# gopi-erabati/SRFDet3D

Measured on AMD Instinct MI355X. Metric: frames/sec, srfdet_voxel_nusc_LC synthetic 30k-pt sweeps, higher is better.
Workload: dtype f32

## Files before the change

include/srfdet3d.h:

```cpp
#ifndef SRFDET3D_H
#define SRFDET3D_H

#include <stddef.h>
#include <stdint.h>

#ifdef __cplusplus
extern "C" {
#endif

typedef void *srf_stream_t;

#define SRF_OK 0
#define SRF_EINVAL (-1)
#define SRF_EWORKSPACE (-2)
#define SRF_EUNSUPPORTED (-3)
#define SRF_EHIP_BASE (-1000)

int srf_abi_version(void);
const char *srf_error_string(int code);
int srf_device_count(void);

size_t srf_bitmap_words(const int *shape, int batch);
size_t srf_bitmap_pair_count_ints(void);
size_t srf_bitmap_workspace_bytes(size_t words);
int srf_bitmap_build(const int *indices, int A, const int *shape, int batch, void *bitmap, int *prefix, int *order,
                     int *sorted_indices, void *workspace, size_t workspace_bytes, srf_stream_t stream);
int srf_bitmap_build_padded(const int *indices, int A, const int *shape, int batch, void *bitmap, int *prefix, int *order,
                            int *sorted_indices, void *workspace, size_t workspace_bytes, srf_stream_t stream);
int srf_bitmap_rulebook_subm(const int *sorted_indices, int A, const int *shape, int batch, const int *ksize,
                             const void *bitmap, const int *prefix, int *nbr , int *pair_counts ,
                             srf_stream_t stream);
int srf_bitmap_strided_outputs(const int *indices, int A, const int *shape, int batch, const int *ksize, const int *stride,
                               const int *pad, void *out_bitmap, int *out_prefix, int *out_indices, int out_capacity,
                               int *num_out, void *workspace, size_t workspace_bytes, srf_stream_t stream);
int srf_bitmap_strided_outputs_static(const int *indices, int A, const int *shape, int batch, const int *ksize, const int *stride,
                                      const int *pad, void *out_bitmap, int *out_prefix, int *out_indices, int out_capacity,
                                      int *num_out, void *workspace, size_t workspace_bytes, srf_stream_t stream);
int srf_bitmap_strided_pairs(const int *out_indices, const int *num_out, int max_out, const int *shape, int batch,
                             const int *ksize, const int *stride, const int *pad, const void *in_bitmap, const int *in_prefix,
                             int in_rows, int *nbr, int nbr_stride, int fill_tail, int *pair_counts, srf_stream_t stream);

int srf_densify_bev(const float *feats, int A, int C, const void *bitmap, const int *prefix, int B, int D, int H, int W, float *out,
                    srf_stream_t stream);

int srf_pillar_vfe(const float *voxels, const int *num, const int *coors4, const int *rows_dev, int rows, int P, int nf,
                   const float *voxel_size , const float *offset , int cluster_center, int voxel_center, int legacy,
                   const float *W, const float *scale, const float *shift, int Cout, float *out, srf_stream_t stream);
// ... 342 lines not shown
```

srfdet3d_amd/_lib.py:

```python
import ctypes
import os
from ctypes import POINTER, c_char_p, c_float, c_int, c_int64, c_longlong, c_size_t, c_void_p

_HERE = os.path.dirname(os.path.abspath(__file__))
LIB_PATH = os.path.join(_HERE, "libsrfdet3d_hip.so")

_lib = None


class FeatMap(ctypes.Structure):
    _fields_ = [("data", c_void_p), ("N", c_int), ("H", c_int), ("W", c_int),
                ("stride_n", c_int64), ("stride_c", c_int64), ("stride_h", c_int64), ("stride_w", c_int64),
                ("spatial_scale", c_float)]


_P = c_void_p
_HF = POINTER(c_float)
_HI = POINTER(c_int)

SIGNATURES = {
    "srf_abi_version": (c_int, []),
    "srf_error_string": (c_char_p, [c_int]),
    "srf_device_count": (c_int, []),
    "srf_points_filter_workspace_bytes": (c_size_t, [c_int]),
# ... 39 lines not shown
    "srf_conv_wgrad_nhwc": (c_int, [_P, c_int64, _P, c_int64, c_int, c_int, c_int, c_int, c_int, c_int, _P, c_size_t, _P, _P]),
    "srf_spconv_tiles_count": (c_int, [c_int]),
    "srf_spconv_tiles_row_cost": (c_int, []),
    "srf_spconv_tiles_workspace_bytes": (c_size_t, [c_int]),
    "srf_spconv_tiles_build": (c_int, [_P, c_int, c_int, c_int, _P, _P, _P, _P]),
    "srf_spconv_order_ints": (c_size_t, [c_int, c_int]),
    "srf_spconv_order_build": (c_int, [_P, c_int, c_int, c_int, _P, _P, _P]),
    "srf_spconv_bf16_packed_weight_bytes": (c_size_t, [c_int, c_int, c_int]),
    "srf_spconv_bf16_pack_weights": (c_int, [_P, c_int, c_int, c_int, _P, _P]),
    "srf_spconv_fwd_bf16": (c_int, [_P, c_int, c_int, _P, c_int, _P, c_int, c_int, c_int, _P, _P, _P, c_int, _P, _P, _P, _P]),
    "srf_densify": (c_int, [_P, _P, c_int, c_int, c_int, c_int, c_int, c_int, _P, c_int, _P]),
    "srf_roi_extract": (c_int, [POINTER(FeatMap), c_int, c_int, _P, c_int, c_int, c_int, c_float, _P, c_int64,
                                c_int64, c_int64, c_int, _P, _P]),
    "srf_roi_extract_sum": (c_int, [POINTER(FeatMap), c_int, c_int, _P, c_int, c_int, c_int, c_int, c_float, _P, c_int64, c_int64, c_int64, _P]),
    "srf_linear_workspace_bytes": (c_size_t, [c_int, c_int, c_int]),
    "srf_linear": (c_int, [_P, c_int, c_int, c_int, _P, c_int, c_int, _P, _P, _P, c_float, c_int, _P, c_int, _P, _P, c_float,
                           c_int, _P, c_int, _P, c_size_t, _P]),
    "srf_self_attention": (c_int, [_P, c_int, c_int, c_int, _P, _P]),
    "srf_self_attention_batched": (c_int, [_P, c_int, c_int, c_int, c_int, _P, _P]),
    "srf_dynconv_mid": (c_int, [_P, _P, c_int, c_int, c_int, c_int, _P, _P, c_float, _P, _P, c_float, _P, _P]),
    "srf_bitmap_words": (c_size_t, [_HI, c_int]),
    "srf_bitmap_pair_count_ints": (c_size_t, []),
    "srf_bitmap_workspace_bytes": (c_size_t, [c_size_t]),
    "srf_bitmap_build": (c_int, [_P, c_int, _HI, c_int, _P, _P, _P, _P, _P, c_size_t, _P]),
    "srf_densify_bev": (c_int, [_P, c_int, c_int, _P, _P, c_int, c_int, c_int, c_int, _P, _P]),
    "srf_pillar_vfe": (c_int, [_P, _P, _P, _P, c_int, c_int, c_int, _HF, _HF, c_int, c_int, c_int, _P, _P, _P, c_int, _P, _P]),
    "srf_pillar_scatter_nhwc": (c_int, [_P, _P, _P, c_int, c_int, c_int, c_int, c_int, _P, _P]),
    "srf_dvfe_workspace_bytes": (c_size_t, [c_int, c_int]),
    "srf_dvfe_fwd": (c_int, [_P, c_int, c_int, _P, _P, _P, _P, _P, _P, c_int, _HF, _HF, c_int, _P, _P, _P, _P, _P, _P, c_int, _P, _P, _P,
                             c_int, _P, _P, _P, c_int, _P, _P, c_size_t, _P]),
    "srf_bitmap_build_padded": (c_int, [_P, c_int, _HI, c_int, _P, _P, _P, _P, _P, c_size_t, _P]),
    "srf_bitmap_rulebook_subm": (c_int, [_P, c_int, _HI, c_int, _HI, _P, _P, _P, _P, _P]),
    "srf_bitmap_strided_outputs": (c_int, [_P, c_int, _HI, c_int, _HI, _HI, _HI, _P, _P, _P, c_int, _P, _P, c_size_t, _P]),
    "srf_bitmap_strided_outputs_static": (c_int, [_P, c_int, _HI, c_int, _HI, _HI, _HI, _P, _P, _P, c_int, _P, _P, c_size_t, _P]),
    "srf_bitmap_strided_pairs": (c_int, [_P, _P, c_int, _HI, c_int, _HI, _HI, _HI, _P, _P, c_int, _P, c_int, c_int, _P, _P]),
    "srf_upsample_add": (c_int, [_P, _P, c_int, c_int, c_int, c_int, c_int, _P, _P]),
    "srf_maxpool3s2_ceil": (c_int, [_P, c_int, c_int, c_int, _P, _P]),
    "srf_ese_gate": (c_int, [_P, c_int, c_int, _P, _P, _P, _P]),
    "srf_nchw_to_nhwc": (c_int, [_P, c_int, c_int, c_int, _P, _P]),
    "srf_dwconv3x3s2": (c_int, [_P, c_int, c_int, c_int, c_int, _P, _P, _P, c_int, _P, _P]),
    "srf_channel_affine": (c_int, [_P, c_int, c_int, c_int, c_longlong, _P, _P, c_int, _P, c_int, _P, c_longlong, _P]),
    "srf_conv1x1_packed_weight_bytes": (c_size_t, [c_int, c_int]),
    "srf_conv1x1_pack_weights": (c_int, [_P, c_int, c_int, _P, _P]),
    "srf_conv1x1": (c_int, [POINTER(c_void_p), _HI, c_int, c_int, c_int, _P, c_int, _P, _P, c_int, _P, _P]),
    "srf_wino43_packed_weight_bytes": (c_size_t, [c_int, c_int]),
    "srf_wino43_pack_weights": (c_int, [_P, c_int, c_int, _P, _P]),
# ... 124 lines not shown
```

srfdet3d_amd/csrc/common.hpp:

```cpp
#pragma once
#include <hip/hip_runtime.h>
#include <stdint.h>
#include <stdlib.h>

#include "../../include/srfdet3d.h"

#define SRF_WAVE 64

#define SRF_HIP_TRY(expr)                                    \
    do {                                                     \
        hipError_t _e = (expr);                              \
        if (_e != hipSuccess) return SRF_EHIP_BASE - (int)_e; \
    } while (0)

#define SRF_LAUNCH_CHECK()                                   \
    do {                                                     \
        hipError_t _e = hipGetLastError();                   \
        if (_e != hipSuccess) return SRF_EHIP_BASE - (int)_e; \
    } while (0)

static inline int srf_ceil_div(long long a, long long b) { return (int)((a + b - 1) / b); }
static inline size_t srf_align256(size_t x) { return (x + 255) & ~(size_t)255; }

static inline long long srf_knob(const char *name, long long dflt)
// ... 107 lines not shown
    return v;
}

__device__ __forceinline__ int srf_block_exclusive_scan_256(int v, int *total, int *lds4 )
{
    const int lane = threadIdx.x & 63, wave = threadIdx.x >> 6;
    int inc = srf_wave_inclusive_scan(v);
    if (lane == 63) lds4[wave] = inc;
    __syncthreads();
    int w0 = lds4[0], w1 = lds4[1], w2 = lds4[2], w3 = lds4[3];
    int base = (wave > 0 ? w0 : 0) + (wave > 1 ? w1 : 0) + (wave > 2 ? w2 : 0);
    *total = w0 + w1 + w2 + w3;
    __syncthreads();
    return base + inc - v;
}

#define SRF_SCAN_THREADS 256
#define SRF_SCAN_ITEMS 8
#define SRF_SCAN_TILE (SRF_SCAN_THREADS * SRF_SCAN_ITEMS)

static inline int srf_scan_blocks(long long n) { return n > 0 ? srf_ceil_div(n, SRF_SCAN_TILE) : 1; }

template <class ValF>
__global__ __launch_bounds__(SRF_SCAN_THREADS) void srf_scan_reduce_k(int n, ValF val, int *__restrict__ partial)
{
    __shared__ int lds[4];
    const int base = blockIdx.x * SRF_SCAN_TILE;
    int s = 0;
#pragma unroll
    for (int j = 0; j < SRF_SCAN_ITEMS; ++j) {
        int i = base + j * SRF_SCAN_THREADS + threadIdx.x;
        if (i < n) s += val(i);
    }
    s = srf_wave_sum(s);
    if ((threadIdx.x & 63) == 0) lds[threadIdx.x >> 6] = s;
    __syncthreads();
    if (threadIdx.x == 0) partial[blockIdx.x] = lds[0] + lds[1] + lds[2] + lds[3];
}

static __global__ __launch_bounds__(256) void srf_scan_partials_k(int nb, int *__restrict__ partial, int *__restrict__ total_out,
                                                         int clamp_max)
{
    __shared__ int lds[4];
    int carry = 0;
    for (int base = 0; base < nb; base += 256) {
        int i = base + threadIdx.x;
        int v = i < nb ? partial[i] : 0;
        int tot;
        int ex = srf_block_exclusive_scan_256(v, &tot, lds);
        if (i < nb) partial[i] = carry + ex;
        carry += tot;
    }
    if (threadIdx.x == 0) {
        partial[nb] = carry;
        if (total_out) *total_out = (clamp_max >= 0 && carry > clamp_max) ? clamp_max : carry;
    }
}

template <class ValF, class OutF>
__global__ __launch_bounds__(SRF_SCAN_THREADS) void srf_scan_apply_k(int n, ValF val, const int *__restrict__ partial,
                                                                   OutF out)
{
    __shared__ int lds[4];
    const int base = blockIdx.x * SRF_SCAN_TILE + threadIdx.x * SRF_SCAN_ITEMS;
    int v[SRF_SCAN_ITEMS];
    int s = 0;
#pragma unroll
    for (int j = 0; j < SRF_SCAN_ITEMS; ++j) {
        int i = base + j;
        v[j] = i < n ? val(i) : 0;
        s += v[j];
    }
    int tot;
    int ex = srf_block_exclusive_scan_256(s, &tot, lds) + partial[blockIdx.x];
#pragma unroll
    for (int j = 0; j < SRF_SCAN_ITEMS; ++j) {
        int i = base + j;
        if (i < n) out(i, v[j], ex);
        ex += v[j];
    }
}

#define SRF_SCAN_SINGLE_THREADS 1024
#define SRF_SCAN_SINGLE_MAX (SRF_SCAN_SINGLE_THREADS * SRF_SCAN_ITEMS)

template <class ValF, class OutF>
__global__ __launch_bounds__(SRF_SCAN_SINGLE_THREADS) void srf_scan_single_k(int n, ValF val, OutF out, int *__restrict__ partial_total,
                                                                           int *__restrict__ total_out, int clamp_max)
{
    __shared__ int s_w[SRF_SCAN_SINGLE_THREADS / 64];
    const int lane = threadIdx.x & 63, wave = threadIdx.x >> 6;
    int carry = 0;
    for (int base0 = 0; base0 < n; base0 += SRF_SCAN_SINGLE_THREADS * SRF_SCAN_ITEMS) {
        const int base = base0 + threadIdx.x * SRF_SCAN_ITEMS;
        int v[SRF_SCAN_ITEMS];
        int s = 0;
#pragma unroll
        for (int j = 0; j < SRF_SCAN_ITEMS; ++j) {
            const int i = base + j;
            v[j] = i < n ? val(i) : 0;
            s += v[j];
        }
        const int inc = srf_wave_inclusive_scan(s);
        if (lane == 63) s_w[wave] = inc;
        __syncthreads();
        int before = 0, tot = 0;
#pragma unroll
        for (int w = 0; w < SRF_SCAN_SINGLE_THREADS / 64; ++w) {
            const int c = s_w[w];
            before += w < wave ? c : 0;
            tot += c;
        }
        __syncthreads();
        int ex = carry + before + inc - s;
#pragma unroll
        for (int j = 0; j < SRF_SCAN_ITEMS; ++j) {
            const int i = base + j;
            if (i < n) out(i, v[j], ex);
            ex += v[j];
        }
        carry += tot;
    }
    if (threadIdx.x == 0) {
        *partial_total = carry;
        if (total_out) *total_out = (clamp_max >= 0 && carry > clamp_max) ? clamp_max : carry;
    }
}

template <class ValF, class OutF>
static inline int srf_device_scan(int n, ValF val, OutF out, int *partial, int *total_out, int clamp_max,
                                  hipStream_t st)
{
    const int nb = srf_scan_blocks(n);
    if (n <= SRF_SCAN_SINGLE_MAX) {
        hipLaunchKernelGGL(HIP_KERNEL_NAME(srf_scan_single_k<ValF, OutF>), dim3(1), dim3(SRF_SCAN_SINGLE_THREADS), 0, st, n, val, out,
                           partial + nb, total_out, clamp_max);
        SRF_LAUNCH_CHECK();
        return SRF_OK;
    }
    hipLaunchKernelGGL(HIP_KERNEL_NAME(srf_scan_reduce_k<ValF>), dim3(nb), dim3(SRF_SCAN_THREADS), 0, st, n, val, partial);
    hipLaunchKernelGGL(srf_scan_partials_k, dim3(1), dim3(256), 0, st, nb, partial, total_out, clamp_max);
    hipLaunchKernelGGL(HIP_KERNEL_NAME(srf_scan_apply_k<ValF, OutF>), dim3(nb), dim3(SRF_SCAN_THREADS), 0, st, n, val,
                       partial, out);
    SRF_LAUNCH_CHECK();
    return SRF_OK;
}
```

srfdet3d_amd/csrc/rulebook.hip:

```cpp
#include "common.hpp"

#define SRF_MAX_K 27

struct ConvGeom {
    int shape[3];
    int oshape[3];
    int ks[3], st[3], pd[3];
    int K;
};

__device__ __forceinline__ uint32_t srf_coord_key(int b, int z, int y, int x, const int *shape)
{
    return (((uint32_t)b * (uint32_t)shape[0] + (uint32_t)z) * (uint32_t)shape[1] + (uint32_t)y) * (uint32_t)shape[2] +
           (uint32_t)x;
}

__global__ __launch_bounds__(256) void srf_table_build_k(const int4 *__restrict__ indices, int A, ConvGeom g,
                                                       uint32_t *keys, int *rows, uint32_t mask)
{
    const int i = blockIdx.x * 256 + threadIdx.x;
    if (i >= A) return;
    int4 c = indices[i];
    int s = srf_table_insert(keys, mask, srf_coord_key(c.x, c.y, c.z, c.w, g.shape));
    if (s >= 0) rows[s] = i;
// ... 46 lines not shown

__global__ __launch_bounds__(256) void srf_strided_insert_k(const int4 *__restrict__ indices, int A, ConvGeom g,
                                                          uint32_t *okeys, uint32_t omask, int *mincand,
                                                          int *__restrict__ cand_slot)
{
    const long long c = (long long)blockIdx.x * 256 + threadIdx.x;
    if (c >= (long long)A * g.K) return;
    const int i = (int)(c / g.K), k = (int)(c % g.K);
    int4 ci = indices[i];
    int q[3];
    int slot = -1;
    if (srf_candidate(ci, k, g, q)) {
        slot = srf_table_insert(okeys, omask, srf_coord_key(ci.x, q[0], q[1], q[2], g.oshape));
        if (slot >= 0) atomicMin(&mincand[slot], (int)c);
    }
    cand_slot[c] = slot;
}

struct StridedFlag {
    const int *cand_slot;
    const int *mincand;
    __device__ int operator()(int c) const
    {
        int s = cand_slot[c];
        return (s >= 0 && mincand[s] == c) ? 1 : 0;
    }
};

struct StridedAssign {
    const int4 *indices;
    const int *cand_slot;
    int *orows;
    int4 *out_indices;
    ConvGeom g;
    __device__ void operator()(int c, int v, int prefix) const
    {
        if (!v) return;
        const int i = c / g.K, k = c % g.K;
        int4 ci = indices[i];
        int q[3];
        srf_candidate(ci, k, g, q);
        orows[cand_slot[c]] = prefix;
        out_indices[prefix] = make_int4(ci.x, q[0], q[1], q[2]);
    }
};

__global__ __launch_bounds__(256) void srf_strided_fill_k(int A, int K, const int *__restrict__ cand_slot,
                                                        const int *__restrict__ orows, int num_out,
// ... 358 lines not shown
        if (v >= in_rows) v = -1;
        nbr[(size_t)k * nbr_stride + o] = v;
    } else if (fill_tail && o < nbr_stride) {
        nbr[(size_t)k * nbr_stride + o] = -1;
    }
    if (pair_counts) srf_bm_count(v >= 0, k, pair_counts);
}

static long long srf_bm_cells(const int *shape, int batch)
{
    if (!shape || batch <= 0 || shape[0] <= 0 || shape[1] <= 0 || shape[2] <= 0) return -1;
    const unsigned long long c = (unsigned long long)batch * shape[0] * shape[1] * shape[2];
    return c < 0xFFFFFFFFull ? (long long)c : -1;
}

extern "C" size_t srf_bitmap_pair_count_ints(void) { return (size_t)SRF_MAX_K * (SRF_BM_REPLICAS + 1); }

extern "C" size_t srf_bitmap_words(const int *shape, int batch)
{
    const long long c = srf_bm_cells(shape, batch);
    return c < 0 ? 0 : (size_t)((c + 31) / 32);
}

extern "C" size_t srf_bitmap_workspace_bytes(size_t words) { return (size_t)(srf_scan_blocks((long long)words) + 1) * sizeof(int); }

static int srf_bitmap_build_impl(const int *indices, int A, const int *shape, int batch, void *bitmap, int *prefix, int *order,
                                 int *sorted_indices, void *workspace, size_t workspace_bytes, srf_stream_t stream, int padded)
{
    const size_t words = srf_bitmap_words(shape, batch);
    if (A < 0 || words == 0 || !bitmap || !prefix || !workspace) return SRF_EINVAL;
    if (workspace_bytes < srf_bitmap_workspace_bytes(words)) return SRF_EWORKSPACE;
    ConvGeom g;
    const int one[3] = {1, 1, 1};
    if (!srf_fill_conv_geom(g, shape, one, one, nullptr, batch)) return SRF_EINVAL;
    hipStream_t st = (hipStream_t)stream;
    SrfFillRegions fill = {};
    fill.ptr[0] = (uint32_t *)bitmap, fill.value[0] = 0u, fill.nwords[0] = words;
    if (padded && A > 0 && order && sorted_indices) {
        fill.ptr[1] = (uint32_t *)order, fill.value[1] = 0u, fill.nwords[1] = (size_t)A;
        fill.ptr[2] = (uint32_t *)sorted_indices, fill.value[2] = 0xFFFFFFFFu, fill.nwords[2] = (size_t)A * 4;
    }
    SRF_HIP_TRY(srf_fill_regions(fill, st));
    if (A > 0) {
        if (!indices) return SRF_EINVAL;
        hipLaunchKernelGGL(srf_bm_mark_k, dim3(srf_ceil_div(A, 256)), dim3(256), 0, st, (const int4 *)indices, A, g,
                           (uint32_t *)bitmap);
    }
    int rc = srf_device_scan((int)words, BmPop{(const uint32_t *)bitmap}, BmPrefix{prefix}, (int *)workspace, nullptr, -1, st);
    if (rc) return rc;
    if (A > 0 && order && sorted_indices)
        hipLaunchKernelGGL(srf_bm_place_k, dim3(srf_ceil_div(A, 256)), dim3(256), 0, st, (const int4 *)indices, A, g,
                           (const uint32_t *)bitmap, prefix, order, (int4 *)sorted_indices);
    SRF_LAUNCH_CHECK();
    return SRF_OK;
}

extern "C" int srf_bitmap_build(const int *indices, int A, const int *shape, int batch, void *bitmap, int *prefix, int *order,
                                int *sorted_indices, void *workspace, size_t workspace_bytes, srf_stream_t stream)
{
    return srf_bitmap_build_impl(indices, A, shape, batch, bitmap, prefix, order, sorted_indices, workspace, workspace_bytes, stream, 0);
}

extern "C" int srf_bitmap_build_padded(const int *indices, int A, const int *shape, int batch, void *bitmap, int *prefix, int *order,
                                       int *sorted_indices, void *workspace, size_t workspace_bytes, srf_stream_t stream)
{
    return srf_bitmap_build_impl(indices, A, shape, batch, bitmap, prefix, order, sorted_indices, workspace, workspace_bytes, stream, 1);
}

extern "C" int srf_bitmap_rulebook_subm(const int *sorted_indices, int A, const int *shape, int batch, const int *ksize,
                                        const void *bitmap, const int *prefix, int *nbr, int *pair_counts, srf_stream_t stream)
{
// ... 10 lines not shown
    if (pair_counts)
        hipLaunchKernelGGL(srf_bm_fold_counts_k, dim3(1), dim3(64), 0, st, pair_counts + SRF_MAX_K, g.K, pair_counts);
    SRF_LAUNCH_CHECK();
    return SRF_OK;
}

static int srf_bitmap_strided_outputs_impl(const int *indices, int A, const int *shape, int batch, const int *ksize,
                                           const int *stride, const int *pad, void *out_bitmap, int *out_prefix, int *out_indices,
                                           int out_capacity, int *num_out, void *workspace, size_t workspace_bytes,
                                           srf_stream_t stream, int fill_tail)
{
    ConvGeom g;
    if (A < 0 || !shape || !ksize || !stride || !pad || !num_out || !out_bitmap || !out_prefix || !workspace || out_capacity < 0)
        return SRF_EINVAL;
    if (!srf_fill_conv_geom(g, shape, ksize, stride, pad, batch)) return SRF_EINVAL;
    const size_t words = srf_bitmap_words(g.oshape, batch);
    if (words == 0) return SRF_EINVAL;
    if (workspace_bytes < srf_bitmap_workspace_bytes(words)) return SRF_EWORKSPACE;
    hipStream_t st = (hipStream_t)stream;
    SrfFillRegions fill = {};
    fill.ptr[0] = (uint32_t *)out_bitmap, fill.value[0] = 0u, fill.nwords[0] = words;
    if (fill_tail && out_indices && out_capacity > 0)
        fill.ptr[1] = (uint32_t *)out_indices, fill.value[1] = 0xFFFFFFFFu, fill.nwords[1] = (size_t)out_capacity * 4;
    SRF_HIP_TRY(srf_fill_regions(fill, st));
    if (A > 0) {
        if (!indices || !out_indices) return SRF_EINVAL;
        hipLaunchKernelGGL(srf_bm_strided_mark_k, dim3(srf_ceil_div(A, 256), g.K), dim3(256), 0, st, (const int4 *)indices, A, g,
                           (uint32_t *)out_bitmap);
    }
    int rc = srf_device_scan((int)words, BmPop{(const uint32_t *)out_bitmap}, BmPrefix{out_prefix}, (int *)workspace, num_out, -1, st);
    if (rc) return rc;
    if (A > 0)
        hipLaunchKernelGGL(srf_bm_emit_k, dim3(srf_ceil_div((long long)words, 256)), dim3(256), 0, st, (const uint32_t *)out_bitmap,
                           out_prefix, (int)words, g.oshape[0], g.oshape[1], g.oshape[2], out_capacity, (int4 *)out_indices);
    SRF_LAUNCH_CHECK();
    return SRF_OK;
}

extern "C" int srf_bitmap_strided_outputs(const int *indices, int A, const int *shape, int batch, const int *ksize,
                                          const int *stride, const int *pad, void *out_bitmap, int *out_prefix, int *out_indices,
                                          int out_capacity, int *num_out, void *workspace, size_t workspace_bytes,
                                          srf_stream_t stream)
{
    return srf_bitmap_strided_outputs_impl(indices, A, shape, batch, ksize, stride, pad, out_bitmap, out_prefix, out_indices,
                                           out_capacity, num_out, workspace, workspace_bytes, stream, 0);
}

extern "C" int srf_bitmap_strided_outputs_static(const int *indices, int A, const int *shape, int batch, const int *ksize,
                                                 const int *stride, const int *pad, void *out_bitmap, int *out_prefix,
                                                 int *out_indices, int out_capacity, int *num_out, void *workspace,
                                                 size_t workspace_bytes, srf_stream_t stream)
{
    return srf_bitmap_strided_outputs_impl(indices, A, shape, batch, ksize, stride, pad, out_bitmap, out_prefix, out_indices,
// ... 59 lines not shown
```

srfdet3d_amd/csrc/scatter.hip:

```cpp
#include "common.hpp"

struct ScatterGeom {
    int D, H, W;
    uint32_t nwords;
};

__device__ __forceinline__ bool srf_coor_key(const int4 &c, const ScatterGeom &g, uint32_t &key)
{
    if (c.x < 0 || c.y < 0 || c.z < 0 || c.w < 0) return false;
    key = (((uint32_t)c.x * (uint32_t)g.D + (uint32_t)c.y) * (uint32_t)g.H + (uint32_t)c.z) * (uint32_t)g.W + (uint32_t)c.w;
    return true;
}

__global__ __launch_bounds__(256) void srf_vu_mark_k(const int4 *__restrict__ coors, int n, ScatterGeom g,
                                                   uint32_t *bitmap)
{
    const int i = blockIdx.x * 256 + threadIdx.x;
    if (i >= n) return;
    uint32_t key;
    if (srf_coor_key(coors[i], g, key)) atomicOr(&bitmap[key >> 5], 1u << (key & 31));
}

struct VuPop {
    const uint32_t *bitmap;
// ... 103 lines not shown
    unsigned long long vol = (unsigned long long)batch;
    for (int d = 0; d < 3; ++d) {
        if (grid_zyx[d] <= 0) return false;
        vol *= (unsigned long long)grid_zyx[d];
    }
    if (vol >= 0xFFFFFFFFull) return false;
    g.D = grid_zyx[0];
    g.H = grid_zyx[1];
    g.W = grid_zyx[2];
    g.nwords = (uint32_t)((vol + 31) / 32);
    return true;
}

static size_t srf_vu_layout(int n, uint32_t nwords, size_t *o_prefix, size_t *o_cursor, size_t *o_partial)
{
    size_t b = srf_align256((size_t)nwords * 4);
    *o_prefix = b;
    b += srf_align256((size_t)nwords * 4);
    *o_cursor = b;
    b += srf_align256((size_t)(n > 0 ? n : 1) * 4);
    *o_partial = b;
    int nb = srf_scan_blocks(nwords);
    int nb2 = srf_scan_blocks(n);
    b += srf_align256((size_t)((nb > nb2 ? nb : nb2) + 1) * 4);
    return b;
}

extern "C" size_t srf_voxel_unique_workspace_bytes(int n, const int *grid_zyx, int batch)
{
    ScatterGeom g;
    if (n < 0 || !srf_scatter_geom(g, grid_zyx, batch)) return 0;
    size_t a, b, c;
    return srf_vu_layout(n, g.nwords, &a, &b, &c);
}

extern "C" int srf_voxel_unique(const int *coors, int n, const int *grid_zyx, int batch, int *out_coors,
                                int *point2voxel, int *counts, int *offsets, int *order, int *num_voxels,
                                void *workspace, size_t workspace_bytes, srf_stream_t stream)
{
    ScatterGeom g;
    if (n < 0 || !srf_scatter_geom(g, grid_zyx, batch) || !num_voxels) return SRF_EINVAL;
    hipStream_t st = (hipStream_t)stream;
    if (n == 0) {
        SRF_HIP_TRY(srf_fill_bytes(num_voxels, 0, sizeof(int), st));
        return SRF_OK;
    }
    if (!coors || !out_coors || !point2voxel || !counts || !offsets || !order || !workspace) return SRF_EINVAL;
    size_t o_prefix, o_cursor, o_partial;
    if (workspace_bytes < srf_vu_layout(n, g.nwords, &o_prefix, &o_cursor, &o_partial)) return SRF_EWORKSPACE;
    uint32_t *bitmap = (uint32_t *)workspace;
    int *prefix = (int *)((char *)workspace + o_prefix);
    int *cursor = (int *)((char *)workspace + o_cursor);
    int *partial = (int *)((char *)workspace + o_partial);

    SRF_HIP_TRY(srf_fill_bytes(bitmap, 0, (size_t)g.nwords * 4, st));
    SRF_HIP_TRY(srf_fill_bytes(cursor, 0, (size_t)n * 4, st));
    SRF_HIP_TRY(srf_fill_bytes(counts, 0, (size_t)n * 4, st));
    const int nblk = srf_ceil_div(n, 256);
    hipLaunchKernelGGL(srf_vu_mark_k, dim3(nblk), dim3(256), 0, st, (const int4 *)coors, n, g, bitmap);
    SRF_LAUNCH_CHECK();
    int rc = srf_device_scan((int)g.nwords, VuPop{bitmap}, VuEmit{bitmap, prefix, (int4 *)out_coors, g}, partial,
                             num_voxels, -1, st);
    if (rc) return rc;
    hipLaunchKernelGGL(srf_vu_map_k, dim3(nblk), dim3(256), 0, st, (const int4 *)coors, n, g, bitmap, prefix, point2voxel,
                       counts);
    SRF_LAUNCH_CHECK();
    rc = srf_device_scan(n, VuCount{counts}, VuOffset{offsets}, partial, nullptr, -1, st);
    if (rc) return rc;
    hipLaunchKernelGGL(srf_vu_place_k, dim3(nblk), dim3(256), 0, st, point2voxel, n, offsets, cursor, order);
    hipLaunchKernelGGL(srf_vu_sort_k, dim3(nblk), dim3(256), 0, st, offsets, counts, num_voxels, order);
    SRF_LAUNCH_CHECK();
    return SRF_OK;
}

extern "C" int srf_scatter_reduce(const float *feats, const int *order, const int *offsets, const int *counts,
                                  const int *num_voxels, int rows, int C, int mode, float *out, srf_stream_t stream)
{
    if (rows < 0 || C <= 0 || (mode != 0 && mode != 1) || !num_voxels) return SRF_EINVAL;
    if (rows == 0) return SRF_OK;
    if (!feats || !order || !offsets || !counts || !out) return SRF_EINVAL;
    hipLaunchKernelGGL(srf_scatter_reduce_k, dim3(srf_ceil_div((long long)rows * C, 256)), dim3(256), 0,
                       (hipStream_t)stream, feats, order, offsets, counts, num_voxels, rows, C, mode, out);
    SRF_LAUNCH_CHECK();
    return SRF_OK;
}
```

srfdet3d_amd/csrc/spconv.hip:

```cpp
#include "common.hpp"

typedef float f32x16 __attribute__((ext_vector_type(16)));
typedef float f32x4 __attribute__((ext_vector_type(4)));

#define SRF_KC 32
#define SRF_KMAX 27

template <int TM, int COUT>
__device__ __forceinline__ void srf_stage_tile(const float *__restrict__ in, int Cin, const float *__restrict__ Wk, int c0,
                                               const int *s_nbr_k, float (*s_a)[SRF_KC + 1], float (*s_w)[COUT])
{
    const int tid = threadIdx.x;
    const bool vec = (Cin & 3) == 0;
    for (int e = tid; e < TM * (SRF_KC / 4); e += 256) {
        const int r = e / (SRF_KC / 4), q = e % (SRF_KC / 4);
        const int i = s_nbr_k[r];
        const int c = c0 + q * 4;
        float4 v = make_float4(0.f, 0.f, 0.f, 0.f);
        if (i >= 0 && c < Cin) {
            const float *src = in + (size_t)i * Cin + c;
            if (vec) {
                v = *reinterpret_cast<const float4 *>(src);
            } else {
                v.x = src[0];
// ... 320 lines not shown
    }
    const int r0 = blockIdx.x * SRF_TB_ROWS;
    int carry = 0;
    for (int j = 0; j < SRF_TB_ROWS / 256; ++j) {
        const int r = r0 + j * 256 + threadIdx.x;
        int c = 0;
        {
            const int rc = r < A ? r : (A > 0 ? A - 1 : 0);
            int v[SRF_KMAX];
#pragma unroll
            for (int k = 0; k < SRF_KMAX; ++k) v[k] = nbr[(size_t)(k < K ? k : K - 1) * nbr_stride + rc];
#pragma unroll
            for (int k = 0; k < SRF_KMAX; ++k) c += (k < K && v[k] >= 0) ? 1 : 0;
            c = r < A ? c + row_cost : 0;
        }
        int total;
        const int ex = srf_block_scan_excl(c, s_scan, total);
        if (r < A) local[r] = carry + ex;
        carry += total;
    }
    if (threadIdx.x == 0) blocksum[blockIdx.x] = carry;
}

__global__ __launch_bounds__(256) void srf_gs_blockscan_k(const int *__restrict__ blocksum, int nb, int *__restrict__ blockoff)
{
    __shared__ int s_scan[4];
    int carry = 0;
    for (int b0 = 0; b0 < nb; b0 += 256) {
        const int b = b0 + threadIdx.x;
        const int v = b < nb ? blocksum[b] : 0;
        int total;
        const int ex = srf_block_scan_excl(v, s_scan, total);
        if (b < nb) blockoff[b] = carry + ex;
        carry += total;
    }
    if (threadIdx.x == 0) blockoff[nb] = carry;
}

__global__ __launch_bounds__(256) void srf_gs_cut_k(const int *__restrict__ local, const int *__restrict__ blockoff, int nb, int A,
                                                  const int *__restrict__ rows_dev, int T, int *__restrict__ tiles)
{
    if (rows_dev) {
        const int live = *rows_dev;
        A = A < live ? A : live;
    }
    const int t = blockIdx.x * 256 + threadIdx.x;
    if (t > T) return;
    const int nbl = (A + SRF_TB_ROWS - 1) / SRF_TB_ROWS;
    if (t == T || A == 0) {
        tiles[t] = A;
        return;
    }
    const long long P = blockoff[nbl];
    const long long target = (P * t + T - 1) / T;
    int lo = 0, hi = nbl - 1;
    while (lo < hi) {
        const int mid = (lo + hi + 1) >> 1;
        if (blockoff[mid] <= target) lo = mid;
        else hi = mid - 1;
    }
    const long long boff = blockoff[lo];
    const int r0 = lo * SRF_TB_ROWS;
    const int r1 = r0 + SRF_TB_ROWS < A ? r0 + SRF_TB_ROWS : A;
    int a = r0, b = r1;
    while (a < b) {
        const int mid = (a + b) >> 1;
        if (boff + local[mid] >= target) b = mid;
        else a = mid + 1;
// ... 1 lines not shown
    tiles[t] = a;
}

extern "C" int srf_spconv_tiles_count(int A_out) { return A_out <= 0 ? 1 : srf_gs_ranges(A_out); }

extern "C" int srf_spconv_tiles_row_cost(void) { return SRF_GS_ROW_BASE; }

extern "C" size_t srf_spconv_tiles_workspace_bytes(int A_out)
{
    if (A_out < 0) return 0;
    const size_t nb = (size_t)(A_out + SRF_TB_ROWS - 1) / SRF_TB_ROWS;
    return ((size_t)A_out + 2 * nb + 8) * sizeof(int);
}

extern "C" int srf_spconv_tiles_build(const int *nbr, int nbr_stride, int K, int A_out, const int *rows_dev, void *workspace,
                                      int *tiles, srf_stream_t stream)
{
    if (A_out < 0 || K <= 0 || K > SRF_KMAX || nbr_stride < A_out || !tiles) return SRF_EINVAL;
    if (A_out > 0 && (!nbr || !workspace)) return SRF_EINVAL;
    hipStream_t st = (hipStream_t)stream;
    const int T = srf_spconv_tiles_count(A_out);
    const int nb = (A_out + SRF_TB_ROWS - 1) / SRF_TB_ROWS;
    int *local = (int *)workspace, *blocksum = local + A_out, *blockoff = blocksum + nb + 1;
    if (nb > 0) {
        hipLaunchKernelGGL(srf_gs_rowpairs_k, dim3(nb), dim3(256), 0, st, nbr, nbr_stride, K, A_out, rows_dev, local, blocksum, SRF_GS_ROW_BASE);
        hipLaunchKernelGGL(srf_gs_blockscan_k, dim3(1), dim3(256), 0, st, blocksum, nb, blockoff);
    }
    hipLaunchKernelGGL(srf_gs_cut_k, dim3(srf_ceil_div(T + 1, 256)), dim3(256), 0, st, local, blockoff, nb, A_out, rows_dev, T, tiles);
    SRF_LAUNCH_CHECK();
    return SRF_OK;
}


typedef __attribute__((address_space(3))) float srf_lds_float;
typedef __attribute__((address_space(3))) f32x4 srf_lds_f32x4;
__device__ __forceinline__ unsigned srf_lds_addr(const void *p) { return (unsigned)(uintptr_t)p; }

struct SrfGspLane {
    unsigned fo0, fo1;
    unsigned sto[4];
    unsigned goff;
    unsigned colbase;
    unsigned boff;
};

struct SrfGspRegs {
    unsigned f0, f1;
    unsigned st[4];
    unsigned gaddr;
    unsigned oaddr[4];
    unsigned pin_addr;
// ... 894 lines not shown
```

srfdet3d_amd/csrc/voxelize.hip:

```cpp
#include "common.hpp"

#define SRF_SENT 0x7F7F7F7F

struct VoxelGeom {
    float vs[3];
    float lo[3];
    int grid[3];
};

__device__ __forceinline__ bool srf_point_coord(const float *p, const VoxelGeom &g, int &cx, int &cy, int &cz)
{
    int c[3];
#pragma unroll
    for (int j = 0; j < 3; ++j) {
        float d = __fsub_rn(p[j], g.lo[j]);
        float q = __fdiv_rn(d, g.vs[j]);
        float f = floorf(q);
        if (!(f >= 0.0f && f < (float)g.grid[j])) return false;
        c[j] = (int)f;
    }
    cx = c[0];
    cy = c[1];
    cz = c[2];
    return true;
// ... 43 lines not shown
    if (srf_point_coord(p, g, cx, cy, cz)) {
        uint32_t key = ((uint32_t)cz * (uint32_t)g.grid[1] + (uint32_t)cy) * (uint32_t)g.grid[0] + (uint32_t)cx;
        slot = srf_table_insert(keys, mask, key);
    }
    pslot[i] = slot;
    if (slot < 0) return;
    atomicMin(&minidx[slot], i);
    int *lst = top + (size_t)slot * max_points;
    if (i < __atomic_load_n(&lst[max_points - 1], __ATOMIC_RELAXED)) {
        int v = i;
        for (int s = 0; s < max_points; ++s) {
            int old = atomicMin(&lst[s], v);
            if (old == SRF_SENT) break;
            v = old > v ? old : v;
        }
    }
}

struct HvFlag {
    const int *pslot;
    const int *minidx;
    __device__ int operator()(int i) const
    {
        int s = pslot[i];
        return (s >= 0 && minidx[s] == i) ? 1 : 0;
    }
};

struct HvAssign {
    const int *pslot;
    const uint32_t *keys;
    int *vox_slot;
    int *coors;
    int max_voxels;
    int gx, gy;
    int cols, batch;
    __device__ void operator()(int i, int v, int prefix) const
    {
        if (!v || prefix >= max_voxels) return;
        int s = pslot[i];
        vox_slot[prefix] = s;
        uint32_t key = keys[s];
        uint32_t x = key % (uint32_t)gx;
        uint32_t t = key / (uint32_t)gx;
        int *c = coors + (size_t)cols * prefix + (cols - 3);
        if (cols == 4) c[-1] = batch;
        c[0] = (int)(t / (uint32_t)gy);
        c[1] = (int)(t % (uint32_t)gy);
// ... 60 lines not shown
                                    const int *grid, int *coors, srf_stream_t stream)
{
    if (n < 0 || nf < 3 || nf > 64 || !vs || !range || !grid) return SRF_EINVAL;
    if (n == 0) return SRF_OK;
    if (!points || !coors) return SRF_EINVAL;
    VoxelGeom g;
    if (!srf_fill_geom(g, vs, range, grid)) return SRF_EINVAL;
    hipLaunchKernelGGL(srf_dynamic_voxelize_k, dim3(srf_ceil_div(n, 256)), dim3(256), 256 * nf * sizeof(float),
                       (hipStream_t)stream, points, n, nf, g, coors);
    SRF_LAUNCH_CHECK();
    return SRF_OK;
}

extern "C" size_t srf_hard_voxelize_workspace_bytes(int n, int max_points)
{
    if (n < 0 || max_points <= 0) return 0;
    size_t cap = (size_t)srf_hv_capacity(n);
    size_t b = 0;
    b += srf_align256(cap * 4);
    b += srf_align256(cap * 4);
    b += srf_align256(cap * (size_t)max_points * 4);
    b += srf_align256((size_t)(n > 0 ? n : 1) * 4);
    b += srf_align256((size_t)(n > 0 ? n : 1) * 4);
    b += srf_align256((size_t)(srf_scan_blocks(n) + 1) * 4);
    return b;
}

static int srf_hard_voxelize_impl(const float *points, int n, int nf, const float *vs, const float *range,
                                  const int *grid, int max_points, int max_voxels, float *voxels, int *coors, int *num,
                                  int *voxel_num, float *mean, int mean_features, void *workspace,
                                  size_t workspace_bytes, srf_stream_t stream, int coor_cols, int batch_index)
{
    if (n < 0 || nf < 3 || nf > 64 || max_points <= 0 || max_points > 64 || max_voxels <= 0 || !vs || !range ||
        !grid || !voxel_num)
        return SRF_EINVAL;
    if (mean && (mean_features <= 0 || mean_features > nf)) return SRF_EINVAL;
    hipStream_t st = (hipStream_t)stream;
    if (n == 0) {
        SRF_HIP_TRY(srf_fill_bytes(voxel_num, 0, sizeof(int), st));
        return SRF_OK;
    }
    if (!points || !voxels || !coors || !num || !workspace) return SRF_EINVAL;
    if (workspace_bytes < srf_hard_voxelize_workspace_bytes(n, max_points)) return SRF_EWORKSPACE;
    VoxelGeom g;
    if (!srf_fill_geom(g, vs, range, grid)) return SRF_EINVAL;

    const size_t cap = (size_t)srf_hv_capacity(n);
    char *w = (char *)workspace;
    uint32_t *keys = (uint32_t *)w;
    w += srf_align256(cap * 4);
    int *minidx = (int *)w;
    w += srf_align256(cap * 4);
    int *top = (int *)w;
    w += srf_align256(cap * (size_t)max_points * 4);
    int *pslot = (int *)w;
    w += srf_align256((size_t)n * 4);
    int *vox_slot = (int *)w;
    w += srf_align256((size_t)n * 4);
    int *partial = (int *)w;

    SrfFillRegions fill = {};
    fill.ptr[0] = keys, fill.value[0] = 0xFFFFFFFFu, fill.nwords[0] = srf_align256(cap * 4) / 4;
    fill.ptr[1] = (uint32_t *)minidx, fill.value[1] = 0x7F7F7F7Fu;
    fill.nwords[1] = (srf_align256(cap * 4) + srf_align256(cap * (size_t)max_points * 4)) / 4;
    SRF_HIP_TRY(srf_fill_regions(fill, st));

    hipLaunchKernelGGL(srf_hv_insert_k, dim3(srf_ceil_div(n, 256)), dim3(256), 256 * nf * sizeof(float), st, points, n,
                       nf, g, max_points, keys, (uint32_t)(cap - 1), minidx, top, pslot);
    SRF_LAUNCH_CHECK();

    HvFlag flag{pslot, minidx};
    HvAssign assign{pslot, keys, vox_slot, coors, max_voxels, grid[0], grid[1], coor_cols, batch_index};
    int rc = srf_device_scan(n, flag, assign, partial, voxel_num, max_voxels, st);
    if (rc) return rc;

    const int rows = n < max_voxels ? n : max_voxels;
    const long long threads = (long long)rows * max_points * nf;
    hipLaunchKernelGGL(srf_hv_gather_k, dim3(srf_ceil_div(threads, 256)), dim3(256), 0, st, points, nf, max_points, top,
                       vox_slot, voxel_num, rows, voxels, num, mean, mean ? mean_features : 0, coor_cols == 4 ? coors : (int *)nullptr);
    SRF_LAUNCH_CHECK();
    return SRF_OK;
}

extern "C" int srf_hard_voxelize(const float *points, int n, int nf, const float *vs, const float *range,
                                 const int *grid, int max_points, int max_voxels, float *voxels, int *coors, int *num,
                                 int *voxel_num, float *mean, int mean_features, void *workspace,
                                 size_t workspace_bytes, srf_stream_t stream)
{
    return srf_hard_voxelize_impl(points, n, nf, vs, range, grid, max_points, max_voxels, voxels, coors, num, voxel_num, mean,
                                  mean_features, workspace, workspace_bytes, stream, 3, 0);
}

extern "C" int srf_hard_voxelize_static(const float *points, int n, int nf, const float *vs, const float *range,
                                        const int *grid, int max_points, int max_voxels, float *voxels, int *coors4, int *num,
                                        int *voxel_num, float *mean, int mean_features, int batch_index, void *workspace,
                                        size_t workspace_bytes, srf_stream_t stream)
// ... 6 lines not shown
```

Before: 30.35.

## Fuse scan reduce and partials via last-block ticket; merge gather-scan cut kernels

Device prefix scans now use a last-block-done atomic ticket so the reduce kernel also scans the block partials, cutting the separate partials launch. A ticket word is added to each scan workspace and cleared in the existing batched fill. The single-block path threshold drops to a tunable, lower default. Other changes: the spconv blockscan and cut kernels are merged, value loads are hoisted branch-free, the partials scan handles several items per thread, and separate memsets are batched into one fill. This trades kernel launches for atomics and redundant per-block scanning work.

```diff
diff --git a/include/srfdet3d.h b/include/srfdet3d.h
--- a/include/srfdet3d.h
+++ b/include/srfdet3d.h
@@ -23,6 +23,8 @@
 size_t srf_bitmap_words(const int *shape, int batch);
 size_t srf_bitmap_pair_count_ints(void);
 size_t srf_bitmap_workspace_bytes(size_t words);
+long long srf_scan_single_max_elements(void);
+int srf_scan_launches(long long n, long long single_max, int has_ticket);
 int srf_bitmap_build(const int *indices, int A, const int *shape, int batch, void *bitmap, int *prefix, int *order,
                      int *sorted_indices, void *workspace, size_t workspace_bytes, srf_stream_t stream);
 int srf_bitmap_build_padded(const int *indices, int A, const int *shape, int batch, void *bitmap, int *prefix, int *order,
diff --git a/srfdet3d_amd/_lib.py b/srfdet3d_amd/_lib.py
--- a/srfdet3d_amd/_lib.py
+++ b/srfdet3d_amd/_lib.py
@@ -85,6 +85,8 @@
     "srf_bitmap_words": (c_size_t, [_HI, c_int]),
     "srf_bitmap_pair_count_ints": (c_size_t, []),
     "srf_bitmap_workspace_bytes": (c_size_t, [c_size_t]),
+    "srf_scan_single_max_elements": (c_longlong, []),
+    "srf_scan_launches": (c_int, [c_longlong, c_longlong, c_int]),
     "srf_bitmap_build": (c_int, [_P, c_int, _HI, c_int, _P, _P, _P, _P, _P, c_size_t, _P]),
     "srf_densify_bev": (c_int, [_P, c_int, c_int, _P, _P, c_int, c_int, c_int, c_int, _P, _P]),
     "srf_pillar_vfe": (c_int, [_P, _P, _P, _P, c_int, c_int, c_int, _HF, _HF, c_int, c_int, c_int, _P, _P, _P, c_int, _P, _P]),
diff --git a/srfdet3d_amd/csrc/common.hpp b/srfdet3d_amd/csrc/common.hpp
--- a/srfdet3d_amd/csrc/common.hpp
+++ b/srfdet3d_amd/csrc/common.hpp
@@ -153,35 +153,89 @@
 static inline int srf_scan_blocks(long long n) { return n > 0 ? srf_ceil_div(n, SRF_SCAN_TILE) : 1; }
 
 template <class ValF>
+__device__ __forceinline__ int srf_scan_block_sum(int n, ValF &val, int *lds4)
+{
+    const int base = blockIdx.x * SRF_SCAN_TILE;
+    int v[SRF_SCAN_ITEMS];
+#pragma unroll
+    for (int j = 0; j < SRF_SCAN_ITEMS; ++j) {
+        const int i = base + j * SRF_SCAN_THREADS + threadIdx.x;
+        v[j] = val(i < n ? i : n - 1);
+    }
+    int s = 0;
+#pragma unroll
+    for (int j = 0; j < SRF_SCAN_ITEMS; ++j) s += (base + j * SRF_SCAN_THREADS + (int)threadIdx.x < n) ? v[j] : 0;
+    s = srf_wave_sum(s);
+    if ((threadIdx.x & 63) == 0) lds4[threadIdx.x >> 6] = s;
+    __syncthreads();
+    return lds4[0] + lds4[1] + lds4[2] + lds4[3];
+}
+
+template <class ValF>
 __global__ __launch_bounds__(SRF_SCAN_THREADS) void srf_scan_reduce_k(int n, ValF val, int *__restrict__ partial)
 {
     __shared__ int lds[4];
-    const int base = blockIdx.x * SRF_SCAN_TILE;
-    int s = 0;
-#pragma unroll
-    for (int j = 0; j < SRF_SCAN_ITEMS; ++j) {
-        int i = base + j * SRF_SCAN_THREADS + threadIdx.x;
-        if (i < n) s += val(i);
-    }
-    s = srf_wave_sum(s);
-    if ((threadIdx.x & 63) == 0) lds[threadIdx.x >> 6] = s;
+    const int s = srf_scan_block_sum(n, val, lds);
+    if (threadIdx.x == 0) partial[blockIdx.x] = s;
+}
+
+template <bool coherent>
+__device__ __forceinline__ int srf_scan_partials_body(int nb, int *partial, int *lds4)
+{
+    int carry = 0;
+    for (int base0 = 0; base0 < nb; base0 += SRF_SCAN_TILE) {
+        const int base = base0 + threadIdx.x * SRF_SCAN_ITEMS;
+        int v[SRF_SCAN_ITEMS];
+#pragma unroll
+        for (int j = 0; j < SRF_SCAN_ITEMS; ++j) {
+            const int *p = partial + (base + j < nb ? base + j : nb - 1);
+            v[j] = coherent ? __hip_atomic_load(p, __ATOMIC_RELAXED, __HIP_MEMORY_SCOPE_AGENT) : *p;
+        }
+        int s = 0;
+#pragma unroll
+        for (int j = 0; j < SRF_SCAN_ITEMS; ++j) {
+            v[j] = base + j < nb ? v[j] : 0;
+            s += v[j];
+        }
+        int tot;
+        int ex = carry + srf_block_exclusive_scan_256(s, &tot, lds4);
+#pragma unroll
+        for (int j = 0; j < SRF_SCAN_ITEMS; ++j) {
+            if (base + j < nb) partial[base + j] = ex;
+            ex += v[j];
+        }
+        carry += tot;
+    }
+    return carry;
+}
+
+template <class ValF>
+__global__ __launch_bounds__(SRF_SCAN_THREADS) void srf_scan_reduce_last_k(int n, ValF val, int *partial, int *ticket,
+                                                                         int *__restrict__ total_out, int clamp_max)
+{
+    __shared__ int lds[5];
+    const int s = srf_scan_block_sum(n, val, lds);
+    if (threadIdx.x == 0) {
+        __hip_atomic_store(partial + blockIdx.x, s, __ATOMIC_RELAXED, __HIP_MEMORY_SCOPE_AGENT);
+        asm volatile("s_waitcnt vmcnt(0)" ::: "memory");
+        const int t = __hip_atomic_fetch_add(ticket, 1, __ATOMIC_RELAXED, __HIP_MEMORY_SCOPE_AGENT);
+        lds[4] = t == (int)gridDim.x - 1;
+    }
     __syncthreads();
-    if (threadIdx.x == 0) partial[blockIdx.x] = lds[0] + lds[1] + lds[2] + lds[3];
-}
-
-static __global__ __launch_bounds__(256) void srf_scan_partials_k(int nb, int *__restrict__ partial, int *__restrict__ total_out,
-                                                         int clamp_max)
+    if (!lds[4]) return;
+    const int nb = (int)gridDim.x;
+    const int carry = srf_scan_partials_body<true>(nb, partial, lds);
+    if (threadIdx.x == 0) {
+        partial[nb] = carry;
+        if (total_out) *total_out = (clamp_max >= 0 && carry > clamp_max) ? clamp_max : carry;
+        __hip_atomic_store(ticket, 0, __ATOMIC_RELAXED, __HIP_MEMORY_SCOPE_AGENT);
+    }
+}
+
+static __global__ __launch_bounds__(256) void srf_scan_partials_k(int nb, int *partial, int *__restrict__ total_out, int clamp_max)
 {
     __shared__ int lds[4];
-    int carry = 0;
-    for (int base = 0; base < nb; base += 256) {
-        int i = base + threadIdx.x;
-        int v = i < nb ? partial[i] : 0;
-        int tot;
-        int ex = srf_block_exclusive_scan_256(v, &tot, lds);
-        if (i < nb) partial[i] = carry + ex;
-        carry += tot;
-    }
+    const int carry = srf_scan_partials_body<false>(nb, partial, lds);
     if (threadIdx.x == 0) {
         partial[nb] = carry;
         if (total_out) *total_out = (clamp_max >= 0 && carry > clamp_max) ? clamp_max : carry;
@@ -197,9 +251,10 @@
     int v[SRF_SCAN_ITEMS];
     int s = 0;
 #pragma unroll
+    for (int j = 0; j < SRF_SCAN_ITEMS; ++j) v[j] = val(base + j < n ? base + j : n - 1);
+#pragma unroll
     for (int j = 0; j < SRF_SCAN_ITEMS; ++j) {
-        int i = base + j;
-        v[j] = i < n ? val(i) : 0;
+        v[j] = base + j < n ? v[j] : 0;
         s += v[j];
     }
     int tot;
@@ -213,7 +268,17 @@
 }
 
 #define SRF_SCAN_SINGLE_THREADS 1024
-#define SRF_SCAN_SINGLE_MAX (SRF_SCAN_SINGLE_THREADS * SRF_SCAN_ITEMS)
+#define SRF_SCAN_SINGLE_ROUND (SRF_SCAN_SINGLE_THREADS * SRF_SCAN_ITEMS)
+#define SRF_SCAN_SINGLE_MAX_DEFAULT (5 * SRF_SCAN_SINGLE_THREADS)
+static inline long long srf_scan_single_max(void)
+{
+    static const long long v = srf_knob("SRF_SCAN_SINGLE_MAX", SRF_SCAN_SINGLE_MAX_DEFAULT);
+    return v < 0 ? 0 : v;
+}
+static inline int srf_scan_launches_for(long long n, long long single_max, int has_ticket)
+{
+    return n <= single_max ? 1 : (has_ticket ? 2 : 3);
+}
 
 template <class ValF, class OutF>
 __global__ __launch_bounds__(SRF_SCAN_SINGLE_THREADS) void srf_scan_single_k(int n, ValF val, OutF out, int *__restrict__ partial_total,
@@ -222,14 +287,15 @@
     __shared__ int s_w[SRF_SCAN_SINGLE_THREADS / 64];
     const int lane = threadIdx.x & 63, wave = threadIdx.x >> 6;
     int carry = 0;
-    for (int base0 = 0; base0 < n; base0 += SRF_SCAN_SINGLE_THREADS * SRF_SCAN_ITEMS) {
+    for (int base0 = 0; base0 < n; base0 += SRF_SCAN_SINGLE_ROUND) {
         const int base = base0 + threadIdx.x * SRF_SCAN_ITEMS;
         int v[SRF_SCAN_ITEMS];
         int s = 0;
 #pragma unroll
-        for (int j = 0; j < SRF_SCAN_ITEMS; ++j) {
-            const int i = base + j;
-            v[j] = i < n ? val(i) : 0;
+        for (int j = 0; j < SRF_SCAN_ITEMS; ++j) v[j] = val(base + j < n ? base + j : n - 1);
+#pragma unroll
+        for (int j = 0; j < SRF_SCAN_ITEMS; ++j) {
+            v[j] = base + j < n ? v[j] : 0;
             s += v[j];
         }
         const int inc = srf_wave_inclusive_scan(s);
@@ -260,17 +326,23 @@
 
 template <class ValF, class OutF>
 static inline int srf_device_scan(int n, ValF val, OutF out, int *partial, int *total_out, int clamp_max,
-                                  hipStream_t st)
+                                  hipStream_t st, int *ticket = nullptr)
 {
     const int nb = srf_scan_blocks(n);
-    if (n <= SRF_SCAN_SINGLE_MAX) {
+    const int launches = srf_scan_launches_for(n, srf_scan_single_max(), ticket != nullptr);
+    if (launches == 1) {
         hipLaunchKernelGGL(HIP_KERNEL_NAME(srf_scan_single_k<ValF, OutF>), dim3(1), dim3(SRF_SCAN_SINGLE_THREADS), 0, st, n, val, out,
                            partial + nb, total_out, clamp_max);
         SRF_LAUNCH_CHECK();
         return SRF_OK;
     }
-    hipLaunchKernelGGL(HIP_KERNEL_NAME(srf_scan_reduce_k<ValF>), dim3(nb), dim3(SRF_SCAN_THREADS), 0, st, n, val, partial);
-    hipLaunchKernelGGL(srf_scan_partials_k, dim3(1), dim3(256), 0, st, nb, partial, total_out, clamp_max);
+    if (launches == 2) {
+        hipLaunchKernelGGL(HIP_KERNEL_NAME(srf_scan_reduce_last_k<ValF>), dim3(nb), dim3(SRF_SCAN_THREADS), 0, st, n, val, partial,
+                           ticket, total_out, clamp_max);
+    } else {
+        hipLaunchKernelGGL(HIP_KERNEL_NAME(srf_scan_reduce_k<ValF>), dim3(nb), dim3(SRF_SCAN_THREADS), 0, st, n, val, partial);
+        hipLaunchKernelGGL(srf_scan_partials_k, dim3(1), dim3(256), 0, st, nb, partial, total_out, clamp_max);
+    }
     hipLaunchKernelGGL(HIP_KERNEL_NAME(srf_scan_apply_k<ValF, OutF>), dim3(nb), dim3(SRF_SCAN_THREADS), 0, st, n, val,
                        partial, out);
     SRF_LAUNCH_CHECK();
diff --git a/srfdet3d_amd/csrc/rulebook.hip b/srfdet3d_amd/csrc/rulebook.hip
--- a/srfdet3d_amd/csrc/rulebook.hip
+++ b/srfdet3d_amd/csrc/rulebook.hip
@@ -92,8 +92,9 @@
     const int *mincand;
     __device__ int operator()(int c) const
     {
-        int s = cand_slot[c];
-        return (s >= 0 && mincand[s] == c) ? 1 : 0;
+        const int s = cand_slot[c];
+        const int m = mincand[s >= 0 ? s : 0];
+        return (s >= 0 && m == c) ? 1 : 0;
     }
 };
 
@@ -498,7 +499,11 @@
     return c < 0 ? 0 : (size_t)((c + 31) / 32);
 }
 
-extern "C" size_t srf_bitmap_workspace_bytes(size_t words) { return (size_t)(srf_scan_blocks((long long)words) + 1) * sizeof(int); }
+extern "C" size_t srf_bitmap_workspace_bytes(size_t words) { return (size_t)(srf_scan_blocks((long long)words) + 2) * sizeof(int); }
+static int *srf_bitmap_ticket(void *workspace, size_t words) { return (int *)workspace + srf_scan_blocks((long long)words) + 1; }
+
+extern "C" long long srf_scan_single_max_elements(void) { return srf_scan_single_max(); }
+extern "C" int srf_scan_launches(long long n, long long single_max, int has_ticket) { return srf_scan_launches_for(n, single_max, has_ticket); }
 
 static int srf_bitmap_build_impl(const int *indices, int A, const int *shape, int batch, void *bitmap, int *prefix, int *order,
                                  int *sorted_indices, void *workspace, size_t workspace_bytes, srf_stream_t stream, int padded)
@@ -516,13 +521,15 @@
         fill.ptr[1] = (uint32_t *)order, fill.value[1] = 0u, fill.nwords[1] = (size_t)A;
         fill.ptr[2] = (uint32_t *)sorted_indices, fill.value[2] = 0xFFFFFFFFu, fill.nwords[2] = (size_t)A * 4;
     }
+    int *ticket = srf_bitmap_ticket(workspace, words);
+    fill.ptr[3] = (uint32_t *)ticket, fill.value[3] = 0u, fill.nwords[3] = 1;
     SRF_HIP_TRY(srf_fill_regions(fill, st));
     if (A > 0) {
         if (!indices) return SRF_EINVAL;
         hipLaunchKernelGGL(srf_bm_mark_k, dim3(srf_ceil_div(A, 256)), dim3(256), 0, st, (const int4 *)indices, A, g,
                            (uint32_t *)bitmap);
     }
-    int rc = srf_device_scan((int)words, BmPop{(const uint32_t *)bitmap}, BmPrefix{prefix}, (int *)workspace, nullptr, -1, st);
+    int rc = srf_device_scan((int)words, BmPop{(const uint32_t *)bitmap}, BmPrefix{prefix}, (int *)workspace, nullptr, -1, st, ticket);
     if (rc) return rc;
     if (A > 0 && order && sorted_indices)
         hipLaunchKernelGGL(srf_bm_place_k, dim3(srf_ceil_div(A, 256)), dim3(256), 0, st, (const int4 *)indices, A, g,
@@ -579,13 +586,15 @@
     fill.ptr[0] = (uint32_t *)out_bitmap, fill.value[0] = 0u, fill.nwords[0] = words;
     if (fill_tail && out_indices && out_capacity > 0)
         fill.ptr[1] = (uint32_t *)out_indices, fill.value[1] = 0xFFFFFFFFu, fill.nwords[1] = (size_t)out_capacity * 4;
+    int *ticket = srf_bitmap_ticket(workspace, words);
+    fill.ptr[2] = (uint32_t *)ticket, fill.value[2] = 0u, fill.nwords[2] = 1;
     SRF_HIP_TRY(srf_fill_regions(fill, st));
     if (A > 0) {
         if (!indices || !out_indices) return SRF_EINVAL;
         hipLaunchKernelGGL(srf_bm_strided_mark_k, dim3(srf_ceil_div(A, 256), g.K), dim3(256), 0, st, (const int4 *)indices, A, g,
                            (uint32_t *)out_bitmap);
     }
-    int rc = srf_device_scan((int)words, BmPop{(const uint32_t *)out_bitmap}, BmPrefix{out_prefix}, (int *)workspace, num_out, -1, st);
+    int rc = srf_device_scan((int)words, BmPop{(const uint32_t *)out_bitmap}, BmPrefix{out_prefix}, (int *)workspace, num_out, -1, st, ticket);
     if (rc) return rc;
     if (A > 0)
         hipLaunchKernelGGL(srf_bm_emit_k, dim3(srf_ceil_div((long long)words, 256)), dim3(256), 0, st, (const uint32_t *)out_bitmap,
diff --git a/srfdet3d_amd/csrc/scatter.hip b/srfdet3d_amd/csrc/scatter.hip
--- a/srfdet3d_amd/csrc/scatter.hip
+++ b/srfdet3d_amd/csrc/scatter.hip
@@ -149,7 +149,7 @@
     *o_partial = b;
     int nb = srf_scan_blocks(nwords);
     int nb2 = srf_scan_blocks(n);
-    b += srf_align256((size_t)((nb > nb2 ? nb : nb2) + 1) * 4);
+    b += srf_align256((size_t)((nb > nb2 ? nb : nb2) + 2) * 4);
     return b;
 }
 
@@ -180,19 +180,24 @@
     int *cursor = (int *)((char *)workspace + o_cursor);
     int *partial = (int *)((char *)workspace + o_partial);
 
-    SRF_HIP_TRY(srf_fill_bytes(bitmap, 0, (size_t)g.nwords * 4, st));
-    SRF_HIP_TRY(srf_fill_bytes(cursor, 0, (size_t)n * 4, st));
-    SRF_HIP_TRY(srf_fill_bytes(counts, 0, (size_t)n * 4, st));
+    const int nb1 = srf_scan_blocks(g.nwords), nb2 = srf_scan_blocks(n);
+    int *ticket = partial + (nb1 > nb2 ? nb1 : nb2) + 1;
+    SrfFillRegions fill = {};
+    fill.ptr[0] = bitmap, fill.value[0] = 0u, fill.nwords[0] = g.nwords;
+    fill.ptr[1] = (uint32_t *)cursor, fill.value[1] = 0u, fill.nwords[1] = (size_t)n;
+    fill.ptr[2] = (uint32_t *)counts, fill.value[2] = 0u, fill.nwords[2] = (size_t)n;
+    fill.ptr[3] = (uint32_t *)ticket, fill.value[3] = 0u, fill.nwords[3] = 1;
+    SRF_HIP_TRY(srf_fill_regions(fill, st));
     const int nblk = srf_ceil_div(n, 256);
     hipLaunchKernelGGL(srf_vu_mark_k, dim3(nblk), dim3(256), 0, st, (const int4 *)coors, n, g, bitmap);
     SRF_LAUNCH_CHECK();
     int rc = srf_device_scan((int)g.nwords, VuPop{bitmap}, VuEmit{bitmap, prefix, (int4 *)out_coors, g}, partial,
-                             num_voxels, -1, st);
+                             num_voxels, -1, st, ticket);
     if (rc) return rc;
     hipLaunchKernelGGL(srf_vu_map_k, dim3(nblk), dim3(256), 0, st, (const int4 *)coors, n, g, bitmap, prefix, point2voxel,
                        counts);
     SRF_LAUNCH_CHECK();
-    rc = srf_device_scan(n, VuCount{counts}, VuOffset{offsets}, partial, nullptr, -1, st);
+    rc = srf_device_scan(n, VuCount{counts}, VuOffset{offsets}, partial, nullptr, -1, st, ticket);
     if (rc) return rc;
     hipLaunchKernelGGL(srf_vu_place_k, dim3(nblk), dim3(256), 0, st, point2voxel, n, offsets, cursor, order);
     hipLaunchKernelGGL(srf_vu_sort_k, dim3(nblk), dim3(256), 0, st, offsets, counts, num_voxels, order);
diff --git a/srfdet3d_amd/csrc/spconv.hip b/srfdet3d_amd/csrc/spconv.hip
--- a/srfdet3d_amd/csrc/spconv.hip
+++ b/srfdet3d_amd/csrc/spconv.hip
@@ -366,28 +366,38 @@
     if (threadIdx.x == 0) blocksum[blockIdx.x] = carry;
 }
 
-__global__ __launch_bounds__(256) void srf_gs_blockscan_k(const int *__restrict__ blocksum, int nb, int *__restrict__ blockoff)
+#define SRF_GS_SCAN_ITEMS 4
+__global__ __launch_bounds__(256) void srf_gs_scan_cut_k(const int *__restrict__ local, const int *__restrict__ blocksum, int *blockoff,
+                                                       int nb, int A, const int *__restrict__ rows_dev, int T, int *__restrict__ tiles)
 {
     __shared__ int s_scan[4];
-    int carry = 0;
-    for (int b0 = 0; b0 < nb; b0 += 256) {
-        const int b = b0 + threadIdx.x;
-        const int v = b < nb ? blocksum[b] : 0;
-        int total;
-        const int ex = srf_block_scan_excl(v, s_scan, total);
-        if (b < nb) blockoff[b] = carry + ex;
-        carry += total;
-    }
-    if (threadIdx.x == 0) blockoff[nb] = carry;
-}
-
-__global__ __launch_bounds__(256) void srf_gs_cut_k(const int *__restrict__ local, const int *__restrict__ blockoff, int nb, int A,
-                                                  const int *__restrict__ rows_dev, int T, int *__restrict__ tiles)
-{
     if (rows_dev) {
         const int live = *rows_dev;
         A = A < live ? A : live;
     }
+    int carry = 0;
+    for (int b0 = 0; b0 < nb; b0 += 256 * SRF_GS_SCAN_ITEMS) {
+        const int b = b0 + threadIdx.x * SRF_GS_SCAN_ITEMS;
+        int v[SRF_GS_SCAN_ITEMS];
+#pragma unroll
+        for (int j = 0; j < SRF_GS_SCAN_ITEMS; ++j) v[j] = blocksum[b + j < nb ? b + j : nb - 1];
+        int s = 0;
+#pragma unroll
+        for (int j = 0; j < SRF_GS_SCAN_ITEMS; ++j) {
+            v[j] = b + j < nb ? v[j] : 0;
+            s += v[j];
+        }
+        int total;
+        int ex = carry + srf_block_scan_excl(s, s_scan, total);
+#pragma unroll
+        for (int j = 0; j < SRF_GS_SCAN_ITEMS; ++j) {
+            if (b + j < nb) blockoff[b + j] = ex;
+            ex += v[j];
+        }
+        carry += total;
+    }
+    if (nb > 0 && threadIdx.x == 0) blockoff[nb] = carry;
+    __syncthreads();
     const int t = blockIdx.x * 256 + threadIdx.x;
     if (t > T) return;
     const int nbl = (A + SRF_TB_ROWS - 1) / SRF_TB_ROWS;
@@ -435,11 +445,9 @@
     const int T = srf_spconv_tiles_count(A_out);
     const int nb = (A_out + SRF_TB_ROWS - 1) / SRF_TB_ROWS;
     int *local = (int *)workspace, *blocksum = local + A_out, *blockoff = blocksum + nb + 1;
-    if (nb > 0) {
+    if (nb > 0)
         hipLaunchKernelGGL(srf_gs_rowpairs_k, dim3(nb), dim3(256), 0, st, nbr, nbr_stride, K, A_out, rows_dev, local, blocksum, SRF_GS_ROW_BASE);
-        hipLaunchKernelGGL(srf_gs_blockscan_k, dim3(1), dim3(256), 0, st, blocksum, nb, blockoff);
-    }
-    hipLaunchKernelGGL(srf_gs_cut_k, dim3(srf_ceil_div(T + 1, 256)), dim3(256), 0, st, local, blockoff, nb, A_out, rows_dev, T, tiles);
+    hipLaunchKernelGGL(srf_gs_scan_cut_k, dim3(srf_ceil_div(T + 1, 256)), dim3(256), 0, st, local, blocksum, blockoff, nb, A_out, rows_dev, T, tiles);
     SRF_LAUNCH_CHECK();
     return SRF_OK;
 }
diff --git a/srfdet3d_amd/csrc/voxelize.hip b/srfdet3d_amd/csrc/voxelize.hip
--- a/srfdet3d_amd/csrc/voxelize.hip
+++ b/srfdet3d_amd/csrc/voxelize.hip
@@ -89,8 +89,9 @@
     const int *minidx;
     __device__ int operator()(int i) const
     {
-        int s = pslot[i];
-        return (s >= 0 && minidx[s] == i) ? 1 : 0;
+        const int s = pslot[i];
+        const int m = minidx[s >= 0 ? s : 0];
+        return (s >= 0 && m == i) ? 1 : 0;
     }
 };
 
@@ -197,7 +198,7 @@
     b += srf_align256(cap * (size_t)max_points * 4);
     b += srf_align256((size_t)(n > 0 ? n : 1) * 4);
     b += srf_align256((size_t)(n > 0 ? n : 1) * 4);
-    b += srf_align256((size_t)(srf_scan_blocks(n) + 1) * 4);
+    b += srf_align256((size_t)(srf_scan_blocks(n) + 2) * 4);
     return b;
 }
 
@@ -233,11 +234,13 @@
     int *vox_slot = (int *)w;
     w += srf_align256((size_t)n * 4);
     int *partial = (int *)w;
+    int *ticket = partial + srf_scan_blocks(n) + 1;
 
     SrfFillRegions fill = {};
     fill.ptr[0] = keys, fill.value[0] = 0xFFFFFFFFu, fill.nwords[0] = srf_align256(cap * 4) / 4;
     fill.ptr[1] = (uint32_t *)minidx, fill.value[1] = 0x7F7F7F7Fu;
     fill.nwords[1] = (srf_align256(cap * 4) + srf_align256(cap * (size_t)max_points * 4)) / 4;
+    fill.ptr[2] = (uint32_t *)ticket, fill.value[2] = 0u, fill.nwords[2] = 1;
     SRF_HIP_TRY(srf_fill_regions(fill, st));
 
     hipLaunchKernelGGL(srf_hv_insert_k, dim3(srf_ceil_div(n, 256)), dim3(256), 256 * nf * sizeof(float), st, points, n,
@@ -246,7 +249,7 @@
 
     HvFlag flag{pslot, minidx};
     HvAssign assign{pslot, keys, vox_slot, coors, max_voxels, grid[0], grid[1], coor_cols, batch_index};
-    int rc = srf_device_scan(n, flag, assign, partial, voxel_num, max_voxels, st);
+    int rc = srf_device_scan(n, flag, assign, partial, voxel_num, max_voxels, st, ticket);
     if (rc) return rc;
 
     const int rows = n < max_voxels ? n : max_voxels;
```

New measurement: 30.34 (median of 2 runs). About the same (-0.0%).
